# ayushpradhan-dev/robust-speech-analysis-framework

Hardware: AMD Instinct MI355X
Metric: audio-seconds processed/sec (extract+CNN-LSTM fwd) (higher is better)
Workload: dtype f32

## Files before the change

robust_speech_analysis_framework_amd/csrc/gemm_f16x3.h:

```cpp
#pragma once
#if defined(__HIPCC__)
#include "gemm_f32.h"
#define H3_HD __host__ __device__ inline
#else
#include <cstdint>
#define H3_HD inline
#endif

namespace rsaf {

struct H3Div { unsigned mul; int shift; };
inline H3Div h3_div_make(int d) {
    int l = 0;
    while ((1LL << l) < d) ++l;
    const uint64_t two = 1ULL << (31 + l);
    H3Div r;
    r.mul = (unsigned)((two + (uint64_t)d - 1) / (uint64_t)d);
    r.shift = 31 + l;
    return r;
}
H3_HD int h3_div(int n, H3Div r) { return (int)(((uint64_t)(unsigned)n * r.mul) >> r.shift); }
inline bool h3_div_check(H3Div r, int d, int nmax) {
    if (d <= 0 || nmax < 0 || (uint64_t)r.mul * (uint64_t)d < (1ULL << r.shift)) return false;
    const int64_t top = (int64_t)(nmax / d) * d;
// ... 17 lines not shown
    int64_t c_plane, ldcp, sCp;
    const float* c_scale;
    int c_scale_zs, c_scale_ms;
    unsigned* amax_out;
    int amax_zs;
    const int* amax_row_slot;
    int amax_col_min;
    const float* bias;
    const float* R;
    int64_t ldr, sR;
    int M, N, K, nz;
    const int64_t* ztab;
    const int* row_tab;
    int act;
    float alpha;
    int group_m;
    int a_panel, b_panel, cp_panel;
    int nz2;
    int64_t sA2, sB2, sC2, sBias2;
    int b_panel_rows;
    int a_panel_rows, a_tap_panels, a_tap_inv;
    int tiles_m, tiles_n, nwg;
    H3Div inv_nwg, inv_nz2, inv_per_group, inv_gsz, inv_gsz_last;
};

struct H3Tile { int z, z1, z2, tm, tn; };
H3_HD H3Tile h3_tile_at(const GemmH3Params& p, int t) {
    H3Tile T;
    T.z = h3_div(t, p.inv_nwg);
    const int orig = t - T.z * p.nwg;
    T.z1 = h3_div(T.z, p.inv_nz2);
    T.z2 = T.z - T.z1 * (p.nz2 > 1 ? p.nz2 : 1);
    const int xcd = orig & 7, q8 = p.nwg >> 3, r8 = p.nwg & 7;
    const int wg = (xcd < r8 ? xcd * (q8 + 1) : r8 * (q8 + 1) + (xcd - r8) * q8) + (orig >> 3);
    const int per_group = p.group_m * p.tiles_n;
    const int grp = h3_div(wg, p.inv_per_group);
    const int first_m = grp * p.group_m;
    const bool full = p.tiles_m - first_m >= p.group_m;
    const int gsz = full ? p.group_m : p.tiles_m - first_m;
    const int in_grp = wg - grp * per_group;
    T.tn = h3_div(in_grp, full ? p.inv_gsz : p.inv_gsz_last);
    T.tm = first_m + (in_grp - T.tn * gsz);
    return T;
}
inline bool h3_grid_fill(GemmH3Params& p, int bm, int bn) {
    const int64_t tn = (p.N + bn - 1) / bn, tm = (p.M + bm - 1) / bm;
    if (tn <= 0 || tm <= 0 || p.nz <= 0 || p.group_m <= 0 || tn * tm * p.nz > 0x7fffffffLL || p.group_m * tn > 0x7fffffffLL) return false;
    p.tiles_m = (int)tm; p.tiles_n = (int)tn; p.nwg = (int)(tm * tn);
    const int nz2 = p.nz2 > 1 ? p.nz2 : 1, per_group = (int)(p.group_m * tn);
    const int last = p.tiles_m % p.group_m ? p.tiles_m % p.group_m : p.group_m;
    p.inv_nwg = h3_div_make(p.nwg); p.inv_nz2 = h3_div_make(nz2); p.inv_per_group = h3_div_make(per_group);
    p.inv_gsz = h3_div_make(p.group_m); p.inv_gsz_last = h3_div_make(last);
    return h3_div_check(p.inv_nwg, p.nwg, (int)(tm * tn * p.nz - 1)) && h3_div_check(p.inv_nz2, nz2, p.nz - 1) &&
           h3_div_check(p.inv_per_group, per_group, p.nwg - 1) && h3_div_check(p.inv_gsz, p.group_m, per_group - 1) &&
           h3_div_check(p.inv_gsz_last, last, per_group - 1);
}

struct H3KStep { int64_t step, jump; int wrap; };
H3_HD H3KStep h3_kstep(int64_t kstride, int tap_panels, int unit) {
    H3KStep s;
    s.step = kstride * unit;
    s.jump = tap_panels > 0 ? (16 - (int64_t)(tap_panels - 1) * kstride) * unit : s.step;
    s.wrap = tap_panels > 0 ? tap_panels : 0x7fffffff;
    return s;
}
H3_HD int64_t h3_kstep_next(const H3KStep& s, int& pc) {
    const bool w = pc + 1 == s.wrap;
    pc = w ? 0 : pc + 1;
    return w ? s.jump : s.step;
}

#if defined(__HIPCC__)
int launch_gemm_f16x3(const GemmH3Params& p, hipStream_t stream, const char* tag);

int launch_f16x2_row_scales(const float* src, int64_t rows, int K, int64_t ld, float* scale, float* norm2, unsigned* stat_max,
                            hipStream_t stream);
int launch_split_f16x2(const float* src, int64_t rows, int K, int64_t ld, const float* scale, int scale_stride, uint16_t* planes,
                       int64_t plane_stride, int panels, hipStream_t stream);
int launch_scale_from_bound(const unsigned* amax_bits, int64_t n, const float* factor_dev, float factor_host, const float* add_dev,
                            float* scale, hipStream_t stream);

H3_HD float f16x2_scale_for_bound(float bound) {
    union { float f; unsigned u; } v;
    v.f = bound;
    const int e = (int)((v.u >> 23) & 0xff);
    if (e == 0) return 1.0f;
// ... 46 lines not shown
```

robust_speech_analysis_framework_amd/csrc/gemm_f16x3.hip:

```cpp
#include <algorithm>
#include <type_traits>

#include "gemm_f16x3.h"

namespace rsaf {

using f32x16 = __attribute__((ext_vector_type(16))) float;
using f16x8 = __attribute__((ext_vector_type(8))) _Float16;
typedef __attribute__((address_space(3))) void* lds_ptr3;
typedef const __attribute__((address_space(1))) void* glb_ptr3;

__device__ __forceinline__ unsigned short f16_bits(_Float16 h) { return __builtin_bit_cast(unsigned short, h); }

__device__ __forceinline__ void split2(float xs, unsigned short& h, unsigned short& l) {
    const _Float16 hh = (_Float16)xs;
    const _Float16 ll = (_Float16)(xs - (float)hh);
    h = f16_bits(hh);
    l = f16_bits(ll);
}

template <int TM_, int TN_, int WM_, int WN_, int NST_, int WGS_>
struct H3Cfg {
    static constexpr int TM = TM_, TN = TN_, WM = WM_, WN = WN_, NST = NST_, WGS = WGS_;
    static constexpr int BM = 32 * TM * WM, BN = 32 * TN * WN, BK = 16, NPL = 2;
// ... 43 lines not shown
            if (T.m0 < T.Mz) {
                T.coff = p.ztab ? p.ztab[2 * W.z1 + 1] : -1;
                T.aoff = W.z1 * p.sA + W.z2 * p.sA2 + (int64_t)T.m0 * (p.a_panel ? 16 : p.lda);
                T.boff = W.z2 * p.sB2 + (int64_t)T.n0 * (p.b_panel ? 16 : p.ldb);
                T.t = t; T.valid = true;
                break;
            }
        }
        return T;
    };

    constexpr int NI = CFG::A_INSTR + CFG::B_INSTR;
    constexpr int IPW = (NI + NW - 1) / NW;
    constexpr int A_SLOTS = CFG::A_INSTR / NW;
    constexpr int LAST_LIVE = NI - NW * (IPW - 1);
    static_assert(CFG::A_INSTR % NW == 0, "a slot is an A or a B instruction for every wave alike");
    static_assert(LAST_LIVE == NW || LAST_LIVE <= NW / 2, "the waves of group B have the same number of DMA instructions");
    const bool last_live = LAST_LIVE == NW || wave < LAST_LIVE;
#define H3_LIVE(i) ((i) < IPW - 1 || last_live)
    const char* src[IPW][NPL];
    unsigned voff[IPW];
    int ldsoff[IPW];
    int pc = 0;
    const H3KStep a_step = h3_kstep(p.a_panel ? (int64_t)(p.a_panel_rows > 0 ? p.a_panel_rows : p.M) * 16 : 16, p.a_tap_panels, 2);
    const int64_t b_step = 2 * (p.b_panel ? (int64_t)(p.b_panel_rows > 0 ? p.b_panel_rows : p.N) * 16 : 16);
#pragma unroll
    for (int i = 0; i < IPW; ++i) {
        const int jj = i < A_SLOTS ? wave + NW * i : wave + NW * i - CFG::A_INSTR;
        ldsoff[i] = i < A_SLOTS ? jj * 512 : NPL * A_PLANE + jj * 512;
    }
    auto set_tile = [&](const Tile& T) {
        pc = 0;
#pragma unroll
        for (int i = 0; i < IPW; ++i) {
            const bool isA = i < A_SLOTS;
            const int jj = isA ? wave + NW * i : wave + NW * i - CFG::A_INSTR;
            const int row = 32 * jj + (lane >> 1);
            const int dch = (lane & 1) ^ ((row >> 3) & 1);
            const int rr = isA ? ((T.m0 + row < T.Mz) ? row : T.Mz - 1 - T.m0)
                               : ((T.n0 + row < p.N) ? row : p.N - 1 - T.n0);
            const int64_t rs = isA ? (p.a_panel ? 16 : p.lda) : (p.b_panel ? 16 : p.ldb);
            voff[i] = 2u * ((unsigned)rr * (unsigned)rs + 8u * dch);
            const unsigned short* base = isA ? p.A + T.aoff : p.B + T.boff;
#pragma unroll
            for (int pl = 0; pl < NPL; ++pl)
                src[i][pl] = reinterpret_cast<const char*>(base + pl * (isA ? p.a_plane : p.b_plane));
        }
// ... 234 lines not shown
                        const gelu_f32x2 g2 = gelu_pair(gelu_f32x2{v[q][j - 1], v[q][j]});
                        v[q][j - 1] = g2.x; v[q][j] = g2.y;
                    }
                    if (ACT != ACT_NONE && (j & 3) == 3) __builtin_amdgcn_sched_barrier(0);
                }
            }
            if (HAS_R && sub < LAST) load_r((sub + 1) / TN, (sub + 1) % TN);
#pragma unroll
            for (int q = 0; q < NQ; ++q) {
                const int row = drow[q];
                const bool ok = c_ok && tm + RPI * q + lr < Mz && (!ROWTAB || row >= 0);
                if (p.amax_out && ok && gc >= p.amax_col_min) {
#pragma unroll
                    for (int j = 0; j < CW; ++j) row_amax[q] = fmaxf(row_amax[q], fabsf(v[q][j]));
                }
                if (ok) {
                    if (OUT_F32 && p.C) *reinterpret_cast<float4*>(p.C + (done.coff >= 0 ? done.coff : z1 * p.sC) + z2 * p.sC2 + (int64_t)row * p.ldc + gc) =
                        make_float4(v[q][0], v[q][1], v[q][2], v[q][3]);
                    if (OUT_PLANES && p.Cp) {
                        const float cs = csc[q];
                        unsigned short hh[CW], ll[CW];
#pragma unroll
                        for (int j = 0; j < CW; ++j) split2(v[q][j] * cs, hh[j], ll[j]);
                        unsigned short* Pt = p.cp_panel ? p.Cp + (int64_t)(gc >> 4) * ((int64_t)p.M * 16) + (int64_t)row * 16 + (gc & 15)
                                                        : p.Cp + z * p.sCp + (int64_t)row * p.ldcp + gc;
                        if (CW == 8) {
                            *reinterpret_cast<uint4*>(Pt) = make_uint4(hh[0] | ((unsigned)hh[1] << 16), hh[2] | ((unsigned)hh[3] << 16),
                                                                      hh[4 % CW] | ((unsigned)hh[5 % CW] << 16), hh[6 % CW] | ((unsigned)hh[7 % CW] << 16));
                            *reinterpret_cast<uint4*>(Pt + p.c_plane) = make_uint4(ll[0] | ((unsigned)ll[1] << 16), ll[2] | ((unsigned)ll[3] << 16),
                                                                                  ll[4 % CW] | ((unsigned)ll[5 % CW] << 16), ll[6 % CW] | ((unsigned)ll[7 % CW] << 16));
                        } else {
                            *reinterpret_cast<uint2*>(Pt) = make_uint2(hh[0] | ((unsigned)hh[1] << 16), hh[2] | ((unsigned)hh[3] << 16));
                            *reinterpret_cast<uint2*>(Pt + p.c_plane) = make_uint2(ll[0] | ((unsigned)ll[1] << 16), ll[2] | ((unsigned)ll[3] << 16));
                        }
                    }
                }
            }
        }
        if (p.amax_out) {
#pragma unroll
            for (int q = 0; q < NQ; ++q) {
                const int row = tm + RPI * q + lr;
                const bool r_ok = row < Mz && (!ROWTAB || drow[q] >= 0);
                const int slot = !r_ok ? -1 : ROWTAB ? tab_slot[wm0 + mt * 32 + RPI * q + lr]
                                                     : (int)(z1 * p.amax_zs) + (p.amax_row_slot ? p.amax_row_slot[row] : 0);
                unsigned long long todo = __ballot(r_ok);
                while (todo) {
                    const int first = __ffsll((long long)todo) - 1;
// ... 115 lines not shown
    return RSAF_OK;
}

int launch_gemm_f16x3(const GemmH3Params& p, hipStream_t stream, const char* tag) {
    RSAF_CHECK_ARG(p.M >= 0 && p.N >= 0 && p.K >= 0 && p.nz >= 0, "negative dimension");
    if (p.M == 0 || p.N == 0 || p.nz == 0) return RSAF_OK;
    RSAF_CHECK_ARG(p.A && p.B && (p.C || p.Cp), "NULL operand");
    RSAF_CHECK_ARG(p.a_scale && p.b_scale && (!p.Cp || p.c_scale), "every plane operand needs its scales");
    RSAF_CHECK_ARG(p.K % 16 == 0 && p.K >= 16, "K must be a positive multiple of 16");
    RSAF_CHECK_ARG(p.N % 16 == 0, "N must be a multiple of 16 (16-byte epilogue stores)");
    RSAF_CHECK_ARG(p.ldc % 8 == 0 && p.ldcp % 8 == 0 && p.ldr % 4 == 0 && p.c_plane % 8 == 0 && p.sC % 4 == 0 && p.sCp % 8 == 0 &&
                   p.sR % 4 == 0 && p.sC2 % 4 == 0, "ldc / ldr / output strides must keep 16-byte alignment");
    RSAF_CHECK_ARG(p.lda % 8 == 0 && p.ldb % 8 == 0 && p.a_plane % 8 == 0 && p.b_plane % 8 == 0 && p.sA % 8 == 0 && p.sA2 % 8 == 0 &&
                   p.sB2 % 8 == 0, "lda, ldb, the plane strides and the batch strides must be multiples of 8 elements");
    RSAF_CHECK_ARG((reinterpret_cast<uintptr_t>(p.A) & 15) == 0 && (reinterpret_cast<uintptr_t>(p.B) & 15) == 0 &&
                   (reinterpret_cast<uintptr_t>(p.b_scale) & 15) == 0 && p.sBias2 % 4 == 0, "A, B and b_scale must be 16-byte aligned");
    RSAF_CHECK_ARG(!p.R || p.ldr > 0, "residual needs ldr");
    RSAF_CHECK_ARG(p.act >= 0 && p.act <= 2, "act must be 0 (none), 1 (gelu) or 2 (silu)");
    RSAF_CHECK_ARG(p.nz <= 65535, "at most 65535 batches per launch");
    RSAF_CHECK_ARG(!p.cp_panel || p.nz == 1, "the panel layout of the plane output is for unbatched operands");
    RSAF_CHECK_ARG(!p.a_panel || p.nz == 1 || p.a_panel_rows > 0, "a batched A in panels needs a_panel_rows");
    RSAF_CHECK_ARG(p.a_tap_panels == 0 || (p.a_panel && p.a_panel_rows > 0 && p.a_tap_panels > 0 && (p.K / 16) % p.a_tap_panels == 0),
                   "a_tap_panels: A in panels with a_panel_rows, K = taps x a_tap_panels x 16");
    RSAF_CHECK_ARG(p.ldc < (1 << 24) && p.ldcp < (1 << 24) && p.ldr < (1 << 24), "leading dimensions must be below 2^24");
    RSAF_CHECK_ARG(!p.R || p.C, "the residual comes with the fp32 output");
    RSAF_CHECK_ARG(!p.row_tab || (p.nz == 1 && !p.ztab && p.nz2 <= 1 && !p.cp_panel && !p.a_panel && !p.amax_row_slot),
                   "a row table: one batch, row-major A and plane output, no ztab / amax_row_slot");
    RSAF_CHECK_ARG(p.nz2 <= 1 || (p.C && !p.Cp && !p.R && (!p.a_panel || p.a_panel_rows > 0) && p.nz % p.nz2 == 0),
                   "two-level batches: fp32 output only, no residual, A row-major or panels with a_panel_rows, nz a multiple of nz2");
    ProfScope prof(tag ? tag : "gemm_f16x3", stream, 2.0 * p.M * (double)p.N * p.K * p.nz, 0.0);
    using CfgA = H3Cfg<4, 2, 2, 4, 3, 1>;
    using CfgN = H3Cfg<2, 1, 4, 2, 3, 1>;
    using CfgM = H3Cfg<4, 2, 4, 2, 3, 1>;
#define H3_LAUNCH_CFG(CFG, ACT, F32, PL, HR, ...)                                                                       \
    do {                                                                                                                \
        RSAF_CHECK_HIP(hipFuncSetAttribute((const void*)gemm_f16x3_kernel<CFG, ACT, F32, PL, HR, ##__VA_ARGS__>,         \
                                           hipFuncAttributeMaxDynamicSharedMemorySize, CFG::LDS_BYTES));                 \
        RSAF_CHECK_ARG(h3_grid_fill(pp, CFG::BM, CFG::BN), "too many tiles");                                           \
        const int64_t tiles = (int64_t)pp.nwg * pp.nz;                                                                  \
        hipLaunchKernelGGL((gemm_f16x3_kernel<CFG, ACT, F32, PL, HR, ##__VA_ARGS__>),                                    \
                           dim3((unsigned)std::min<int64_t>(tiles, persistent_wgs)), dim3(CFG::THREADS), CFG::LDS_BYTES, stream, pp); \
    } while (0)
#define H3_LAUNCH(ACT, F32, PL, HR, ...)                                                                                \
    do {                                                                                                                \
        if (p.N <= 64) H3_LAUNCH_CFG(CfgN, ACT, F32, PL, HR, ##__VA_ARGS__);                                             \
        else H3_LAUNCH_CFG(CfgA, ACT, F32, PL, HR, ##__VA_ARGS__);                                                       \
    } while (0)
#define H3_LAUNCH3(ACT, F32, PL, HR)                                                                                    \
    do {                                                                                                                \
        if (p.N <= 64) H3_LAUNCH_CFG(CfgN, ACT, F32, PL, HR);                                                            \
// ... 74 lines not shown
```

robust_speech_analysis_framework_amd/csrc/w2v2.hip:

```cpp
#include "w2v2_forward.h"

namespace rsaf {
namespace w2v2 {

int Forward::gemm3(const GemmA& A, const GemmB& B, const Out& o, int M, int N, int K, int nz, const int64_t* zt) {
    GemmH3Params p{};
    p.a_panel = A.panel; p.b_panel = 1; p.cp_panel = o.cp_panel;
    p.A = A.planes; p.a_plane = A.plane; p.lda = A.lda; p.sA = A.sA; p.a_scale = A.scale; p.a_scale_zs = A.scale_zs; p.a_scale_ms = A.scale_ms;
    p.B = B.planes; p.b_plane = (int64_t)N * K; p.ldb = 16; p.b_scale = B.scale;
    p.C = o.Cf; p.ldc = N; p.sC = o.sC;
    p.Cp = o.Cp; p.c_plane = o.c_plane; p.ldcp = N; p.sCp = o.sCp; p.c_scale = o.c_scale; p.c_scale_zs = o.cs_zs; p.c_scale_ms = o.cs_ms;
    p.amax_out = o.amax; p.amax_zs = o.amax_zs; p.amax_row_slot = o.amax_row_slot; p.amax_col_min = o.amax_col_min;
    p.bias = o.bias; p.R = o.R; p.ldr = N; p.sR = o.sC;
    p.M = M; p.N = N; p.K = K; p.nz = nz; p.ztab = zt; p.row_tab = o.row_tab; p.act = o.act; p.alpha = 1.0f; p.group_m = 0;
    return launch_gemm_f16x3(p, s, "w2v2_gemm");
}
GemmA Forward::rows_a(int64_t planes_off, int K, const float* row_scale) const {
    GemmA A;
    A.planes = planes_at(planes_off); A.plane = rows * K; A.lda = K; A.scale = row_scale; A.scale_ms = 1; A.panel = true;
    return A;
}
GemmA Forward::conv_a(const uint16_t* planes, int i) const {
    GemmA A;
    A.planes = planes; A.plane = (int64_t)G * T[i - 1] * C; A.lda = (int64_t)STRD[i] * C; A.sA = (int64_t)T[i - 1] * C;
    A.scale = cscale + (int64_t)(i - 1) * G; A.scale_zs = 1;
    return A;
}
GemmA Forward::conv_a_packed(const uint16_t* planes, int64_t plane, int i) const {
    GemmA A;
    A.planes = planes; A.plane = plane; A.lda = (int64_t)STRD[i] * C;
    A.scale = cscale + (int64_t)(i - 1) * G;
    return A;
}
GemmB Forward::weights_b(int64_t planes_off, int64_t scale_off) const { return GemmB{planes_at(planes_off), ws + scale_off}; }

int Forward::split_wp(int64_t src_off, int64_t nrows, int K, int64_t dst_off, int64_t scale_off, int stat_idx) {
    RSAF_TRY(launch_f16x2_row_scales(Wt + src_off, nrows, K, K, ws + scale_off, nullptr, wstat(stat_idx), s));
    return launch_split_f16x2(Wt + src_off, nrows, K, K, ws + scale_off, 1, planes_at(dst_off), nrows * K, 1, s);
}
int Forward::weight_planes() {
    RSAF_CHECK_HIP(hipMemsetAsync(ws + W.wstat, 0, sizeof(float) * 2 * (WSTAT_LAYER0 + WSTAT_PER_LAYER * c.L), s));
    for (int i = 0; i < 6; ++i)
        RSAF_TRY(split_wp(L.conv[i], C, KERN[i + 1] * C, W.wp_conv[i], W.ws_conv[i], wstat_conv(i)));
    RSAF_TRY(split_wp(L.fpw, Hd, C, W.wp_fp, W.ws_fp, WSTAT_FP));
    if (c.pos_depth() ? posstack_on_mfma(c) : posconv_on_f16x3(c)) {
        RSAF_TRY(split_wp(L.posw, Hd, c.PK * (Hd / c.PG), W.wp_pos, W.ws_pos, WSTAT_POS));
    }
    for (size_t i = 0; i < W.wp_stack.size(); ++i) {
        const int K = c.PK * (Hd / c.PG);
        RSAF_TRY(launch_f16x2_row_scales(Wt + L.stackw[i], Hd, K, K, ws + W.ws_stack[i], nullptr, nullptr, s));
        RSAF_TRY(launch_split_f16x2(Wt + L.stackw[i], Hd, K, K, ws + W.ws_stack[i], 1, planes_at(W.wp_stack[i]), (int64_t)Hd * K, 1, s));
    }
    for (int l = 0; l < c.L; ++l) {
        const LayerOff& lo = L.layers[l];
// ... 195 lines not shown
```

robust_speech_analysis_framework_amd/csrc/w2v2_feat.hip:

```cpp
#include "w2v2_forward.h"
#include "gn_stats.h"

namespace rsaf {
namespace w2v2 {

__global__ __launch_bounds__(256) void w2v2_tables_kernel(const int* __restrict__ len, int n, int C, int Hd, int* __restrict__ Tw,
                                                          int64_t* __restrict__ row0, int64_t* __restrict__ ztab) {
    for (int w = threadIdx.x; w < n; w += 256) {
        int m = len[w];
        for (int i = 0; i < 7; ++i) { m = m >= KERN[i] ? (m - KERN[i]) / STRD[i] + 1 : 0; Tw[(int64_t)i * n + w] = m; }
    }
    __syncthreads();
    if (threadIdx.x == 0) {
        int64_t r = 0;
        for (int w = 0; w < n; ++w) { row0[w] = r; r += Tw[(int64_t)6 * n + w]; }
        row0[n] = r;
    }
    __syncthreads();
    for (int w = threadIdx.x; w < n; w += 256) {
        for (int j = 0; j < 5; ++j) { ztab[((int64_t)j * n + w) * 2] = Tw[(int64_t)(j + 1) * n + w]; ztab[((int64_t)j * n + w) * 2 + 1] = -1; }
        ztab[((int64_t)5 * n + w) * 2] = Tw[(int64_t)6 * n + w]; ztab[((int64_t)5 * n + w) * 2 + 1] = row0[w] * C;
        ztab[((int64_t)6 * n + w) * 2] = Tw[(int64_t)6 * n + w]; ztab[((int64_t)6 * n + w) * 2 + 1] = row0[w] * Hd;
    }
}
// ... 114 lines not shown
            const int64_t o = (2 * (int64_t)out_off[chunk] + t) * C + ch[0];
            if (CPT % 2 == 0) {
#pragma unroll
                for (int k = 0; k < CPT; k += 2) {
                    *reinterpret_cast<unsigned*>(outp + o + k) = hh[k] | ((unsigned)hh[k + 1] << 16);
                    *reinterpret_cast<unsigned*>(outp + plane + o + k) = ll[k] | ((unsigned)ll[k + 1] << 16);
                }
            } else {
#pragma unroll
                for (int k = 0; k < CPT; ++k) { outp[o + k] = hh[k]; outp[plane + o + k] = ll[k]; }
            }
        }
    }
    if (!APPLY) {
#pragma unroll
        for (int k = 0; k < CPT; ++k) {
            part[(((int64_t)chunk * slabs + sl) * 3 + 0) * C + ch[k]] = s[k];
            part[(((int64_t)chunk * slabs + sl) * 3 + 1) * C + ch[k]] = q[k];
            part[(((int64_t)chunk * slabs + sl) * 3 + 2) * C + ch[k]] = mx[k];
        }
    }
}

__global__ __launch_bounds__(384) void lnconv_scale_kernel(const float* __restrict__ cln, int C, int G, float* __restrict__ scale) {
    const int i = threadIdx.x >> 6, lane = threadIdx.x & 63;
    const float* g = cln + (int64_t)2 * i * C;
    const float* b = g + C;
    float mg = 0.f, mb = 0.f;
    for (int c = lane; c < C; c += 64) { mg = fmaxf(mg, fabsf(g[c])); mb = fmaxf(mb, fabsf(b[c])); }
#pragma unroll
    for (int o = 32; o >= 1; o >>= 1) { mg = fmaxf(mg, __shfl_xor(mg, o, 64)); mb = fmaxf(mb, __shfl_xor(mb, o, 64)); }
    const float bound = fmaxf(mg * sqrtf((float)C) * 1.0001f + mb, 0.17f) * 1.0001f;
    const float sc = f16x2_scale_for_bound(bound);
    for (int w = lane; w < G; w += 64) scale[(int64_t)i * G + w] = sc;
}

__global__ __launch_bounds__(64) void conv_bias_max_kernel(const float* __restrict__ cb, int C, float* __restrict__ out) {
    for (int i = 1; i < 6; ++i) {
        float m = 0.f;
        for (int c = threadIdx.x; c < C; c += 64) m = fmaxf(m, fabsf(cb[(int64_t)i * C + c]));
#pragma unroll
        for (int o = 32; o >= 1; o >>= 1) m = fmaxf(m, __shfl_xor(m, o, 64));
        if (threadIdx.x == 0) out[i] = m * 1.000001f;
    }
}

// ... 139 lines not shown
#pragma unroll
        for (int j = 0; j < 10; ++j) wr[j] = w0[c * 10 + j];
        const float bi = cb ? cb[c] : 0.f;
        gn::Sums64 acc;
        for (int t = 0; t < T0; ++t) {
            float y = 0.f;
#pragma unroll
            for (int j = 0; j < 10; ++j) y = fmaf(wr[j], x[5 * t + j], y);
            if (cb) y += bi;
            acc.add(y);
        }
        m = gn::moments_of_sums(acc.s, acc.q, T0);
    }
    float af, bf;
    gn::coefficients(m, g[c], be[c], af, bf);
    ab[((int64_t)chunk * 2 + 0) * C + c] = af;
    ab[((int64_t)chunk * 2 + 1) * C + c] = bf;
    atomicMax(amax + chunk, __float_as_uint((fabsf(af) * mx + fabsf(bf)) * 1.000001f));
}

template <bool APPLY>
static int conv0_launch(const Cfg& c, const float* xn, const float* w0, const float* cb, float* part, const float* ab, const float* scale,
                        unsigned short* outp, int64_t plane, int n, int len, const int* T0w, const int* out_off, int T0, int slab, int slabs,
                        hipStream_t s) {
    const int threads = c.C <= 256 ? c.C : 256;
    const int cpt = c.C / threads;
    dim3 grid((unsigned)slabs, (unsigned)n);
    ProfScope prof(APPLY ? "w2v2_conv0_apply" : "w2v2_conv0_stats", s, 0.0,
                   APPLY ? (double)n * ((double)c.C * T0 * 4.0 + 4.0 * (5.0 * T0 + 5.0)) : (double)n * 4.0 * (5.0 * T0 + 5.0));
#define RSAF_C0K(CPT, BIAS)                                                                                \
    hipLaunchKernelGGL((conv0_kernel<CPT, APPLY, BIAS>), grid, dim3(threads), 0, s, xn, w0, cb, part, ab, scale, outp, plane, len, T0w, \
                       out_off, c.C, slab, slabs)
#define RSAF_C0(BIAS)                                                                                      \
    switch (cpt) {                                                                                         \
        case 1: RSAF_C0K(1, BIAS); break;                                                                  \
        case 2: RSAF_C0K(2, BIAS); break;                                                                  \
        case 3: RSAF_C0K(3, BIAS); break;                                                                  \
        case 4: RSAF_C0K(4, BIAS); break;                                                                  \
        default: set_error("conv0: unsupported conv_dim"); return RSAF_ERR_ARG;                            \
    }
    if (cb) { RSAF_C0(true) } else { RSAF_C0(false) }
#undef RSAF_C0
#undef RSAF_C0K
    RSAF_CHECK_HIP(hipGetLastError());
    return RSAF_OK;
}

static int conv0_ln_launch(const Cfg& c, const float* xn, const float* w0, const float* cb, const float* lg, const float* lb,
                           const float* scale, unsigned short* outp, int64_t plane, int n, int len, const int* T0w, int T0,
                           int T0g, hipStream_t s) {
    constexpr int FR = 64;
    dim3 grid((unsigned)((T0g + FR - 1) / FR), (unsigned)n);
    ProfScope prof("w2v2_conv0_ln", s, 0.0, (double)n * ((double)c.C * T0g * 4.0 + 4.0 * (5.0 * T0g + 5.0)));
    const int cpt = (c.C + 63) / 64;
#define RSAF_C0L(CPT)                                                                                                      \
    hipLaunchKernelGGL((conv0_ln_kernel<CPT>), grid, dim3(256), 0, s, xn, w0, cb, lg, lb, scale, outp, plane, len, T0w, T0, \
                       c.C, FR)
    switch (cpt) {
        case 1: RSAF_C0L(1); break;
        case 2: RSAF_C0L(2); break;
        case 3: RSAF_C0L(3); break;
        case 4: RSAF_C0L(4); break;
        case 8: RSAF_C0L(8); break;
        case 12: RSAF_C0L(12); break;
// ... 63 lines not shown
            hipLaunchKernelGGL(conv_ln_gelu_kernel, dim3((unsigned)((lrows + 3) / 4)), dim3(256), 0, s, ws + W.Q,
                               cln + (int64_t)2 * i * C, cln + (int64_t)(2 * i + 1) * C, cscale + (int64_t)i * G,
                               planes_at(W.P), (int64_t)G * T[i] * C, lrows, T[i], Tw + (int64_t)i * n + g0, C);
            RSAF_CHECK_HIP(hipGetLastError());
        }
    }
    return RSAF_OK;
}
int Forward::convs_group_norm(int g0, int g, const int* Tg) {
    int64_t M[7] = {};
    for (int w = g0; w < g0 + g; ++w) {
        int Tw_[7];
        chunk_lengths(R.len[w], Tw_);
        for (int i = 1; i < 7; ++i) M[i] += Tw_[i] + 1;
    }
    RSAF_CHECK_ARG(2 * M[1] + 1 < 0x7fffffffLL && rows < 0x7fffffffLL, "too many conv rows in one group");
    PackBases bases{};
    for (int i = 1; i < 7; ++i) bases.b[i] = packed_tab_base(G, T, i);
    hipLaunchKernelGGL(w2v2_pack_offsets_kernel, dim3(1), dim3(64), 0, s, Tw + g0, n, g, G, coff);
    hipLaunchKernelGGL(w2v2_pack_rows_kernel, dim3(g, 6), dim3(256), 0, s, Tw + g0, n, G, coff, row0 + g0, crow, bases);
    RSAF_CHECK_HIP(hipGetLastError());
    const int slabs_g = (Tg[0] + STAT_SLAB - 1) / STAT_SLAB;
    RSAF_TRY(conv0_launch<false>(c, ws + W.xn, Wt + L.conv0, cbias, ws + W.part, nullptr, nullptr, nullptr, 0, g, R.maxlen, Tw + g0,
                                  nullptr, T[0], STAT_SLAB, slabs_g, s));
    const int64_t tot = (int64_t)g * C;
    hipLaunchKernelGGL(gn_finalize_kernel, dim3((unsigned)((tot + 255) / 256)), dim3(256), 0, s, ws + W.part,
                       Wt + L.gng, Wt + L.gnb, ws + W.ab, camax, g, C, slabs_g, Tw + g0, ws + W.xn, R.maxlen, Wt + L.conv0, cbias);
    RSAF_CHECK_HIP(hipGetLastError());
    RSAF_TRY(launch_scale_from_bound(camax, g, nullptr, 1.0f, nullptr, cscale, s));
    const int slab = 128;
    const int64_t plane_p = p_rows(G, T) * C, plane_q = q_rows(G, T) * C;
    RSAF_TRY(conv0_launch<true>(c, ws + W.xn, Wt + L.conv0, cbias, nullptr, ws + W.ab, cscale, planes_at(W.P), plane_p, g,
                                 R.maxlen, Tw + g0, coff + (G + 1), T[0], slab, (Tg[0] + slab - 1) / slab, s));
    uint16_t* cur = planes_at(W.P);
    uint16_t* nxt = planes_at(W.Q);
    int64_t plane_cur = plane_p, plane_nxt = plane_q;
    for (int i = 1; i < 7; ++i) {
        Out o;
        o.act = ACT_GELU;
        o.row_tab = crow + 2 * bases.b[i];
        if (i < 6) {
            RSAF_TRY(launch_scale_from_bound(camax + (int64_t)(i - 1) * G, g, reinterpret_cast<const float*>(wstat(wstat_conv(i - 1))),
                                              sqrtf((float)(KERN[i] * C)) * 1.00001f, conv_bias ? cb_max + i : nullptr,
                                              cscale + (int64_t)i * G, s));
            o.Cp = nxt; o.c_plane = plane_nxt;
            o.c_scale = cscale + (int64_t)i * G;
            o.amax = camax + (int64_t)i * G;
        } else {
            o.Cf = ws + W.c6;
        }
        o.bias = conv_bias ? cbias + (int64_t)i * C : nullptr;
        RSAF_TRY(gemm3(conv_a_packed(cur, plane_cur, i), weights_b(W.wp_conv[i - 1], W.ws_conv[i - 1]), o, (int)M[i], C, KERN[i] * C));
        std::swap(cur, nxt);
        std::swap(plane_cur, plane_nxt);
    }
    return RSAF_OK;
}

int Forward::feature_projection() {
    RSAF_CHECK_HIP(hipMemsetAsync(ws + W.fp_amax, 0, sizeof(unsigned) * n, s));
    LnArgs a;
    a.x = ws + W.c6; a.g = Wt + L.fplg; a.b = Wt + L.fplb;
    a.planes = planes_at(W.lnfp); a.panel = true; a.scale_out = ws + W.s_lnfp;
    if (layer_norm) {
        a.var = 2; a.pg = cln + (int64_t)12 * C; a.pb = cln + (int64_t)13 * C;
    } else if (c.flags & F_NO_FEAT_PROJ_LN) {
        a.var = 3;
    }
    RSAF_TRY(ln(a, rows, C, c.eps, s));
    Out o;
    o.Cf = x; o.bias = Wt + L.fpb;
    o.amax = bits_at(W.fp_amax); o.amax_row_slot = rowwin;
    return gemm3(rows_a(W.lnfp, C, ws + W.s_lnfp), weights_b(W.wp_fp, W.ws_fp), o, (int)rows, Hd, C);
}

// ... 3 lines not shown
```

robust_speech_analysis_framework_amd/csrc/w2v2_forward.h:

```cpp
#pragma once
#include <algorithm>
#include <cstdlib>
#include <vector>

#include "gemm_f32.h"
#include "gemm_f16x3.h"
#include "w2v2_layout.h"

namespace rsaf {
namespace w2v2 {

__device__ __forceinline__ unsigned short f16_bits_w(_Float16 h) { return __builtin_bit_cast(unsigned short, h); }
__device__ __forceinline__ void split2_w(float xs, unsigned short& h, unsigned short& l) {
    const _Float16 hh = (_Float16)xs;
    h = f16_bits_w(hh);
    l = f16_bits_w((_Float16)(xs - (float)hh));
}

#define RSAF_TRY(expr) do { const int rc_ = (expr); if (rc_) return rc_; } while (0)

struct LnArgs {
    const float *x = nullptr, *r = nullptr;
    const float *g = nullptr, *b = nullptr;
    float* out = nullptr;
// ... 2 lines not shown
    const int64_t* row0 = nullptr;
    unsigned short* planes = nullptr;
    bool panel = false;
    float* scale_out = nullptr;
    const unsigned *bound_w = nullptr, *bound_b = nullptr;
    float* bound_scale_out = nullptr;
    unsigned* win_norm = nullptr;
    int var = 0;
    const float *pg = nullptr, *pb = nullptr;
    float* aux = nullptr;
    float* tap = nullptr;
    int tap_mode = 0;
    const int64_t* tap_row_start = nullptr;
};

int ln(const LnArgs& a, int64_t rows, int D, float eps, hipStream_t s);

struct GemmA {
    const uint16_t* planes = nullptr;
    int64_t plane = 0, lda = 0, sA = 0;
    const float* scale = nullptr;
    int scale_zs = 0, scale_ms = 0;
    bool panel = false;
};
struct GemmB {
    const uint16_t* planes = nullptr;
    const float* scale = nullptr;
};
struct Out {
    const float* bias = nullptr;
    const float* R = nullptr;
    int act = ACT_NONE;
    float* Cf = nullptr;
    int64_t sC = 0;
    uint16_t* Cp = nullptr;
    int64_t c_plane = 0, sCp = 0;
    const float* c_scale = nullptr;
    int cs_zs = 0, cs_ms = 0;
    bool cp_panel = false;
    unsigned* amax = nullptr;
    int amax_zs = 0;
    const int* amax_row_slot = nullptr;
    int amax_col_min = 0;
    const int* row_tab = nullptr;
};

struct Forward {
    const Cfg& c;
    const Rag& R;
    const Layout L;
    const Workspace& W;
    const float* Wt;
    float* ws;
    hipStream_t s;
    const float* wav = nullptr;
    const int64_t* chunk_start = nullptr;
    float* out = nullptr;
    const int64_t* out_row_start = nullptr;
    float* const* taps = nullptr;
    const int n, C, Hd, Tt, G, hd;
    const int* T;
    const int64_t rows;
// ... 14 lines not shown
    float* x;

    Forward(const Cfg& c_, const Rag& R_, const Workspace& W_, const float* weights, void* workspace, hipStream_t s_)
        : c(c_), R(R_), L(make_layout(c_)), W(W_), Wt(weights), ws(static_cast<float*>(workspace)), s(s_), n(R_.n), C(c_.C), Hd(c_.Hd),
          Tt(R_.Tmax[6]), G(conv_group(R_.n)), hd(c_.Hd / c_.NH), T(R_.Tmax), rows(R_.rows), scale(1.0f / sqrtf((float)hd)),
          fused(fused_attention(c_, Tt)), relpos(c_.flags & F_REL_POS_BIAS), pre_ln(c_.flags & F_PRE_LN),
          layer_norm(c_.flags & F_LAYER_FEAT_NORM), conv_bias(c_.flags & F_CONV_BIAS),
          Tw(reinterpret_cast<int*>(ws + W.t_Tw)), row0(reinterpret_cast<int64_t*>(ws + W.t_row0)),
          ztab(reinterpret_cast<int64_t*>(ws + W.t_ztab)), rowwin(reinterpret_cast<int*>(ws + W.t_rowwin)),
          coff(reinterpret_cast<int*>(ws + W.t_coff)), crow(reinterpret_cast<int*>(ws + W.t_crow)),
          cscale(ws + W.conv_scale), camax(bits_at(W.conv_amax)), cbias(conv_bias ? Wt + L.cb : nullptr), cln(Wt + L.cln),
          cb_max(conv_bias ? ws + W.cb_max : nullptr), x(ws + W.x) {}

    uint16_t* planes_at(int64_t off) const { return reinterpret_cast<uint16_t*>(ws + off); }
    unsigned* bits_at(int64_t off) const { return reinterpret_cast<unsigned*>(ws + off); }
    unsigned* wstat(int idx) const { return bits_at(W.wstat) + 2 * idx; }
    float* tap(int k) const { return taps ? taps[k] : nullptr; }
    float* gate_rows() const { return relpos ? ws + W.att : nullptr; }
    float* gate() const { return relpos ? ws + W.gate : nullptr; }
    const float* reltab() const { return relpos ? Wt + L.reltab : nullptr; }

    int gemm3(const GemmA& A, const GemmB& B, const Out& o, int M, int N, int K, int nz = 1, const int64_t* zt = nullptr);
    GemmA rows_a(int64_t planes_off, int K, const float* row_scale) const, conv_a(const uint16_t* planes, int i) const,
        conv_a_packed(const uint16_t* planes, int64_t plane, int i) const;
    GemmB weights_b(int64_t planes_off, int64_t scale_off) const;
    int split_wp(int64_t src_off, int64_t nrows, int K, int64_t dst_off, int64_t scale_off, int stat_idx), weight_planes();
    int window_tables(const int* len_dev), feature_encoder(), conv_gemm(int i, const uint16_t* a_planes, Out& o, int g0, int g, const int* Tg),
        convs_layer_norm(int g0, int g, const int* Tg), convs_group_norm(int g0, int g, const int* Tg), feature_projection();
    int positional_conv(), positional_conv_stack(), posstack_mfma(int D), posstack_fp32(int D), posconv_regroup_planes(), posconv_lds(),
        posconv_batched_gemm(),
        conv_runs_fp32(const float* src, const float* w, const float* bias, int act, const char* gemm_family, const char* regroup_family);
    template <int MODE> int posstack_rows(const float* src, float* dst);
    template <int NT> int posstack_conv_launch(int i);
    template <int NT, int SP> int posconv_lds_launch();
    int ln_to_qkv(const float* src, const float* res, const float* g, const float* b, float* dst, int k, bool next, float* sum = nullptr);
    int qkv_projection(int l), attention(), attention_three_launch(), out_projection(int l),
        ln_to_ffn(int l, const float* g, const float* b, float* dst), feed_forward(int l, float* dst, const float* res), layer_post_ln(int l),
        layer_pre_ln(int l), encoder_layer(int l);
    template <bool RP> int attention_fused();
};

}
}
```

robust_speech_analysis_framework_amd/csrc/w2v2_layout.h:

```cpp
#pragma once
#include <cstddef>
#include <cstdint>
#include <utility>
#include <vector>

#include "rsaf.h"

#if defined(__HIPCC__)
#define WL_HD __host__ __device__ __forceinline__
#else
#define WL_HD inline
#endif

namespace rsaf {
namespace w2v2 {

constexpr int F_LAYER_FEAT_NORM = RSAF_W2V2_LAYER_FEAT_NORM, F_CONV_BIAS = RSAF_W2V2_CONV_BIAS, F_PRE_LN = RSAF_W2V2_PRE_LN,
              F_NO_INPUT_NORM = RSAF_W2V2_NO_INPUT_NORM, F_NO_FEAT_PROJ_LN = RSAF_W2V2_NO_FEAT_PROJ_LN,
              F_REL_POS_BIAS = RSAF_W2V2_REL_POS_BIAS, F_POS_CONV_STACK = RSAF_W2V2_POS_CONV_STACK,
              F_POS_DEPTH_MASK = RSAF_W2V2_POS_DEPTH_MASK,
              F_ALL = 15 | F_NO_FEAT_PROJ_LN | F_REL_POS_BIAS | F_POS_CONV_STACK | F_POS_DEPTH_MASK;
constexpr int REL_SPAN = RSAF_W2V2_REL_SPAN, REL_TAB = 2 * REL_SPAN - 1;

struct Cfg {
// ... 97 lines not shown
    std::vector<int64_t> wp_qkv, wp_o, wp_1, wp_2;
    int64_t ws_conv[6], ws_fp, ws_pos, wstat;
    std::vector<int64_t> ws_qkv, ws_o, ws_1, ws_2;
    int64_t conv_scale, conv_amax, pos_scale, fp_amax, wlen, win_norm, s_lnfp, s_x, s_ffn, s_att, s_qkv;
    int64_t cb_max;
    int64_t gate;
    std::vector<int64_t> wp_stack, ws_stack;
    int64_t t_Tw, t_row0, t_ztab, t_rowwin;
    int64_t t_coff, t_crow;
};
constexpr int STAT_SLAB = 512;
constexpr int CONV_GROUP = 512;

inline int conv_group(int n) { return n < CONV_GROUP ? n : CONV_GROUP; }
inline bool fused_attention(const Cfg& c, int Tt) { return c.Hd / c.NH == 64 && Tt <= 256; }
inline bool posconv_on_f16x3(const Cfg& c) { return (c.Hd / c.PG) % 16 == 0; }
inline bool posstack_on_mfma(const Cfg& c) { return c.pos_depth() > 0 && (c.Hd / c.PG) % 16 == 0 && c.Hd / c.PG <= 64; }

inline int64_t planes_floats(int64_t n) { return pad4(n); }

inline int64_t packed_in_rows(int G, int Ti) { return 2 * (int64_t)G * (Ti + 1) + 1; }
inline int64_t p_rows(int G, const int* T) { return packed_in_rows(G, T[1]); }
inline int64_t q_rows(int G, const int* T) { return packed_in_rows(G, T[2]); }
inline int64_t packed_tab_base(int G, const int* T, int i) {
    int64_t b = 0;
    for (int j = 1; j < i; ++j) b += (int64_t)G * (T[j] + 1);
    return b;
}

inline int wstat_conv(int i) { return i; }
constexpr int WSTAT_FP = 6, WSTAT_POS = 7, WSTAT_LAYER0 = 8, WSTAT_PER_LAYER = 6;

struct Rag {
    int n = 0, maxlen = 0, Tmax[7] = {};
    int64_t rows = 0;
    std::vector<int> len;
    std::vector<int64_t> row0;
    std::vector<std::pair<int, int>> tgroups;
    std::vector<int> T6;
};

inline const char* make_rag(const int* len_host, int n, int len, Rag& R) {
    R.n = n;
    if (len_host) R.len.assign(len_host, len_host + n);
    else R.len.assign((size_t)n, len);
    R.row0.assign(n + 1, 0);
// ... 113 lines not shown
```

Baseline: 12550.

## Store feature-encoder conv activations as even/odd panel images for strided conv GEMMs

Switches the f16x3 plane layout of the strided feature-encoder convolutions from row-major packed rows to a 16-wide panel layout split into even-row and odd-row images. The GEMM epilogue writes the next layer's A operand directly in this layout, and the A loader's k-step walks across two (or three) taps over the image pair, so the stride-2 conv A tiles become contiguous panel loads. Conv layers after the first use the new layout by default. An opt-in conv0 kernel, enabled by an environment variable, stages outputs in LDS and writes the panels itself. This adds layout complexity and argument checks, and carries a risk of indexing mistakes with odd T lengths.

```diff
diff --git a/robust_speech_analysis_framework_amd/csrc/gemm_f16x3.h b/robust_speech_analysis_framework_amd/csrc/gemm_f16x3.h
--- a/robust_speech_analysis_framework_amd/csrc/gemm_f16x3.h
+++ b/robust_speech_analysis_framework_amd/csrc/gemm_f16x3.h
@@ -63,7 +63,12 @@
     int a_panel_rows, a_tap_panels, a_tap_inv;
     int tiles_m, tiles_n, nwg;
     H3Div inv_nwg, inv_nz2, inv_per_group, inv_gsz, inv_gsz_last;
+    int a_evenodd, cp_evenodd_rows;
 };
+
+H3_HD int64_t h3_evenodd_at(int64_t R, int P, int r, int k) {
+    return (((int64_t)(r & 1) * P + (k >> 4)) * R + (r >> 1)) * 16 + (k & 15);
+}
 
 struct H3Tile { int z, z1, z2, tm, tn; };
 H3_HD H3Tile h3_tile_at(const GemmH3Params& p, int t) {
@@ -98,11 +103,12 @@
 }
 
 struct H3KStep { int64_t step, jump; int wrap; };
-H3_HD H3KStep h3_kstep(int64_t kstride, int tap_panels, int unit) {
+H3_HD H3KStep h3_kstep(int64_t kstride, int tap_panels, int unit, int images = 1) {
     H3KStep s;
+    const int per_wrap = tap_panels * images;
     s.step = kstride * unit;
-    s.jump = tap_panels > 0 ? (16 - (int64_t)(tap_panels - 1) * kstride) * unit : s.step;
-    s.wrap = tap_panels > 0 ? tap_panels : 0x7fffffff;
+    s.jump = tap_panels > 0 ? (16 - (int64_t)(per_wrap - 1) * kstride) * unit : s.step;
+    s.wrap = tap_panels > 0 ? per_wrap : 0x7fffffff;
     return s;
 }
 H3_HD int64_t h3_kstep_next(const H3KStep& s, int& pc) {
diff --git a/robust_speech_analysis_framework_amd/csrc/gemm_f16x3.hip b/robust_speech_analysis_framework_amd/csrc/gemm_f16x3.hip
--- a/robust_speech_analysis_framework_amd/csrc/gemm_f16x3.hip
+++ b/robust_speech_analysis_framework_amd/csrc/gemm_f16x3.hip
@@ -89,7 +89,8 @@
     unsigned voff[IPW];
     int ldsoff[IPW];
     int pc = 0;
-    const H3KStep a_step = h3_kstep(p.a_panel ? (int64_t)(p.a_panel_rows > 0 ? p.a_panel_rows : p.M) * 16 : 16, p.a_tap_panels, 2);
+    const H3KStep a_step = h3_kstep(p.a_panel ? (int64_t)(p.a_panel_rows > 0 ? p.a_panel_rows : p.M) * 16 : 16, p.a_tap_panels, 2,
+                                    (ROWTAB && p.a_evenodd) ? 2 : 1);
     const int64_t b_step = 2 * (p.b_panel ? (int64_t)(p.b_panel_rows > 0 ? p.b_panel_rows : p.N) * 16 : 16);
 #pragma unroll
     for (int i = 0; i < IPW; ++i) {
@@ -370,8 +371,9 @@
                         unsigned short hh[CW], ll[CW];
 #pragma unroll
                         for (int j = 0; j < CW; ++j) split2(v[q][j] * cs, hh[j], ll[j]);
-                        unsigned short* Pt = p.cp_panel ? p.Cp + (int64_t)(gc >> 4) * ((int64_t)p.M * 16) + (int64_t)row * 16 + (gc & 15)
-                                                        : p.Cp + z * p.sCp + (int64_t)row * p.ldcp + gc;
+                        unsigned short* Pt = (ROWTAB && p.cp_panel) ? p.Cp + h3_evenodd_at(p.cp_evenodd_rows, p.N >> 4, row, gc)
+                                             : p.cp_panel ? p.Cp + (int64_t)(gc >> 4) * ((int64_t)p.M * 16) + (int64_t)row * 16 + (gc & 15)
+                                                          : p.Cp + z * p.sCp + (int64_t)row * p.ldcp + gc;
                         if (CW == 8) {
                             *reinterpret_cast<uint4*>(Pt) = make_uint4(hh[0] | ((unsigned)hh[1] << 16), hh[2] | ((unsigned)hh[3] << 16),
                                                                       hh[4 % CW] | ((unsigned)hh[5 % CW] << 16), hh[6 % CW] | ((unsigned)hh[7 % CW] << 16));
@@ -533,10 +535,15 @@
     RSAF_CHECK_ARG(!p.a_panel || p.nz == 1 || p.a_panel_rows > 0, "a batched A in panels needs a_panel_rows");
     RSAF_CHECK_ARG(p.a_tap_panels == 0 || (p.a_panel && p.a_panel_rows > 0 && p.a_tap_panels > 0 && (p.K / 16) % p.a_tap_panels == 0),
                    "a_tap_panels: A in panels with a_panel_rows, K = taps x a_tap_panels x 16");
+    RSAF_CHECK_ARG(!p.a_evenodd || (p.row_tab && p.a_tap_panels > 0 && (p.K / 16 == 2 * p.a_tap_panels || p.K / 16 == 3 * p.a_tap_panels) &&
+                                    p.M <= p.a_panel_rows),
+                   "a_evenodd: a row table, A as two images of a_tap_panels panels x a_panel_rows >= M rows, 2 or 3 taps");
+    RSAF_CHECK_ARG(p.cp_evenodd_rows >= 0 && (p.cp_evenodd_rows > 0) == (p.row_tab && p.cp_panel && p.Cp),
+                   "cp_evenodd_rows comes with a row table and the panel layout of the plane output, and they with it");
     RSAF_CHECK_ARG(p.ldc < (1 << 24) && p.ldcp < (1 << 24) && p.ldr < (1 << 24), "leading dimensions must be below 2^24");
     RSAF_CHECK_ARG(!p.R || p.C, "the residual comes with the fp32 output");
-    RSAF_CHECK_ARG(!p.row_tab || (p.nz == 1 && !p.ztab && p.nz2 <= 1 && !p.cp_panel && !p.a_panel && !p.amax_row_slot),
-                   "a row table: one batch, row-major A and plane output, no ztab / amax_row_slot");
+    RSAF_CHECK_ARG(!p.row_tab || (p.nz == 1 && !p.ztab && p.nz2 <= 1 && (!p.a_panel || p.a_evenodd) && !p.amax_row_slot),
+                   "a row table: one batch, A row-major or an even / odd image pair, no ztab / amax_row_slot");
     RSAF_CHECK_ARG(p.nz2 <= 1 || (p.C && !p.Cp && !p.R && (!p.a_panel || p.a_panel_rows > 0) && p.nz % p.nz2 == 0),
                    "two-level batches: fp32 output only, no residual, A row-major or panels with a_panel_rows, nz a multiple of nz2");
     ProfScope prof(tag ? tag : "gemm_f16x3", stream, 2.0 * p.M * (double)p.N * p.K * p.nz, 0.0);
diff --git a/robust_speech_analysis_framework_amd/csrc/w2v2.hip b/robust_speech_analysis_framework_amd/csrc/w2v2.hip
--- a/robust_speech_analysis_framework_amd/csrc/w2v2.hip
+++ b/robust_speech_analysis_framework_amd/csrc/w2v2.hip
@@ -13,6 +13,8 @@
     p.amax_out = o.amax; p.amax_zs = o.amax_zs; p.amax_row_slot = o.amax_row_slot; p.amax_col_min = o.amax_col_min;
     p.bias = o.bias; p.R = o.R; p.ldr = N; p.sR = o.sC;
     p.M = M; p.N = N; p.K = K; p.nz = nz; p.ztab = zt; p.row_tab = o.row_tab; p.act = o.act; p.alpha = 1.0f; p.group_m = 0;
+    if (A.evenodd_rows > 0) { p.a_evenodd = 1; p.a_panel_rows = A.evenodd_rows; p.a_tap_panels = A.evenodd_panels; }
+    p.cp_evenodd_rows = o.cp_evenodd_rows;
     return launch_gemm_f16x3(p, s, "w2v2_gemm");
 }
 GemmA Forward::rows_a(int64_t planes_off, int K, const float* row_scale) const {
@@ -26,10 +28,11 @@
     A.scale = cscale + (int64_t)(i - 1) * G; A.scale_zs = 1;
     return A;
 }
-GemmA Forward::conv_a_packed(const uint16_t* planes, int64_t plane, int i) const {
+GemmA Forward::conv_a_packed(const uint16_t* planes, int64_t plane, int i, bool evenodd) const {
     GemmA A;
     A.planes = planes; A.plane = plane; A.lda = (int64_t)STRD[i] * C;
     A.scale = cscale + (int64_t)(i - 1) * G;
+    if (evenodd) { A.panel = true; A.lda = 16; A.evenodd_rows = (int)evenodd_img_rows(G, T[i]); A.evenodd_panels = C / 16; }
     return A;
 }
 GemmB Forward::weights_b(int64_t planes_off, int64_t scale_off) const { return GemmB{planes_at(planes_off), ws + scale_off}; }
diff --git a/robust_speech_analysis_framework_amd/csrc/w2v2_feat.hip b/robust_speech_analysis_framework_amd/csrc/w2v2_feat.hip
--- a/robust_speech_analysis_framework_amd/csrc/w2v2_feat.hip
+++ b/robust_speech_analysis_framework_amd/csrc/w2v2_feat.hip
@@ -160,6 +160,69 @@
     }
 }
 
+constexpr int C0P_CH = 128, C0P_FR = 64, C0P_ROWB = C0P_CH * 2 + 16;
+template <bool BIAS>
+__global__ __launch_bounds__(256) void conv0_panels_kernel(const float* __restrict__ xn, const float* __restrict__ w0,
+                                                           const float* __restrict__ cb, const float* __restrict__ ab,
+                                                           const float* __restrict__ scale, unsigned short* __restrict__ outp,
+                                                           int64_t plane, int len, const int* __restrict__ T0w,
+                                                           const int* __restrict__ out_off, int C, int slab, int rimg) {
+    __shared__ __attribute__((aligned(16))) unsigned char stage[2 * C0P_FR * C0P_ROWB];
+    const int chunk = blockIdx.y, lane = threadIdx.x & 63, wave = __builtin_amdgcn_readfirstlane(threadIdx.x >> 6);
+    const int t0 = blockIdx.x * slab, t1 = min(T0w[chunk], t0 + slab);
+    const int c0 = blockIdx.z * C0P_CH, nch = min(C - c0, C0P_CH);
+    const bool live = 2 * lane < nch;
+    const int ch = c0 + (live ? 2 * lane : 0);
+    const float* __restrict__ x = xn + (int64_t)chunk * len;
+    float wr[2][10], a[2], b[2], bi[2];
+    const float sc = scale[chunk];
+#pragma unroll
+    for (int k = 0; k < 2; ++k) {
+#pragma unroll
+        for (int j = 0; j < 10; ++j) wr[k][j] = w0[(ch + k) * 10 + j];
+        bi[k] = BIAS ? cb[ch + k] : 0.f;
+        a[k] = ab[((int64_t)chunk * 2 + 0) * C + ch + k]; b[k] = ab[((int64_t)chunk * 2 + 1) * C + ch + k];
+    }
+    const int np = nch >> 4;
+    const int64_t r0 = 2 * (int64_t)out_off[chunk];
+    const int rr = lane >> 1, half = lane & 1;
+    const int lane_src = 2 * rr * C0P_ROWB + 16 * half, lane_dst = 16 * rr + 8 * half;
+    for (int tb = t0; tb < t1; tb += C0P_FR) {
+        for (int tt = 16 * wave; tt < 16 * wave + 16 && tb + tt < t1; ++tt) {
+            const int t = tb + tt;
+            float xv[10], gv[2];
+#pragma unroll
+            for (int j = 0; j < 10; ++j) xv[j] = x[5 * t + j];
+#pragma unroll
+            for (int k = 0; k < 2; ++k) {
+                float y = 0.f;
+#pragma unroll
+                for (int j = 0; j < 10; ++j) y = fmaf(wr[k][j], xv[j], y);
+                if (BIAS) y += bi[k];
+                gv[k] = fmaf(y, a[k], b[k]);
+            }
+            const gelu_f32x2 g2 = gelu_pair(gelu_f32x2{gv[0], gv[1]});
+            unsigned short hh[2], ll[2];
+            split2_w(g2.x * sc, hh[0], ll[0]);
+            split2_w(g2.y * sc, hh[1], ll[1]);
+            if (live) {
+                *reinterpret_cast<unsigned*>(stage + tt * C0P_ROWB + 4 * lane) = hh[0] | ((unsigned)hh[1] << 16);
+                *reinterpret_cast<unsigned*>(stage + (C0P_FR + tt) * C0P_ROWB + 4 * lane) = ll[0] | ((unsigned)ll[1] << 16);
+            }
+        }
+        __syncthreads();
+#pragma unroll
+        for (int w = 0; w < 4; ++w) {
+            const int img = w & 1, pl = w >> 1;
+            if (tb + 2 * rr + img < t1)
+                for (int panel = wave; panel < np; panel += 4)
+                    *reinterpret_cast<uint4*>(outp + pl * plane + evenodd_at(rimg, C, r0 + tb + img, c0 + 16 * panel) + lane_dst) =
+                        *reinterpret_cast<const uint4*>(stage + (pl * C0P_FR + img) * C0P_ROWB + 32 * panel + lane_src);
+        }
+        __syncthreads();
+    }
+}
+
 __global__ __launch_bounds__(384) void lnconv_scale_kernel(const float* __restrict__ cln, int C, int G, float* __restrict__ scale) {
     const int i = threadIdx.x >> 6, lane = threadIdx.x & 63;
     const float* g = cln + (int64_t)2 * i * C;
@@ -345,7 +408,7 @@
 template <bool APPLY>
 static int conv0_launch(const Cfg& c, const float* xn, const float* w0, const float* cb, float* part, const float* ab, const float* scale,
                         unsigned short* outp, int64_t plane, int n, int len, const int* T0w, const int* out_off, int T0, int slab, int slabs,
-                        hipStream_t s) {
+                        int rimg, hipStream_t s) {
     const int threads = c.C <= 256 ? c.C : 256;
     const int cpt = c.C / threads;
     dim3 grid((unsigned)slabs, (unsigned)n);
@@ -362,7 +425,11 @@
         case 4: RSAF_C0K(4, BIAS); break;                                                                  \
         default: set_error("conv0: unsupported conv_dim"); return RSAF_ERR_ARG;                            \
     }
-    if (cb) { RSAF_C0(true) } else { RSAF_C0(false) }
+    if (APPLY && rimg > 0) {
+        dim3 pgrid((unsigned)slabs, (unsigned)n, (unsigned)((c.C + C0P_CH - 1) / C0P_CH));
+        if (cb) hipLaunchKernelGGL(conv0_panels_kernel<true>, pgrid, dim3(256), 0, s, xn, w0, cb, ab, scale, outp, plane, len, T0w, out_off, c.C, slab, rimg);
+        else hipLaunchKernelGGL(conv0_panels_kernel<false>, pgrid, dim3(256), 0, s, xn, w0, cb, ab, scale, outp, plane, len, T0w, out_off, c.C, slab, rimg);
+    } else if (cb) { RSAF_C0(true) } else { RSAF_C0(false) }
 #undef RSAF_C0
 #undef RSAF_C0K
     RSAF_CHECK_HIP(hipGetLastError());
@@ -472,16 +539,19 @@
     RSAF_CHECK_HIP(hipGetLastError());
     const int slabs_g = (Tg[0] + STAT_SLAB - 1) / STAT_SLAB;
     RSAF_TRY(conv0_launch<false>(c, ws + W.xn, Wt + L.conv0, cbias, ws + W.part, nullptr, nullptr, nullptr, 0, g, R.maxlen, Tw + g0,
-                                  nullptr, T[0], STAT_SLAB, slabs_g, s));
+                                  nullptr, T[0], STAT_SLAB, slabs_g, 0, s));
     const int64_t tot = (int64_t)g * C;
     hipLaunchKernelGGL(gn_finalize_kernel, dim3((unsigned)((tot + 255) / 256)), dim3(256), 0, s, ws + W.part,
                        Wt + L.gng, Wt + L.gnb, ws + W.ab, camax, g, C, slabs_g, Tw + g0, ws + W.xn, R.maxlen, Wt + L.conv0, cbias);
     RSAF_CHECK_HIP(hipGetLastError());
     RSAF_TRY(launch_scale_from_bound(camax, g, nullptr, 1.0f, nullptr, cscale, s));
-    const int slab = 128;
     const int64_t plane_p = p_rows(G, T) * C, plane_q = q_rows(G, T) * C;
+    const auto env1 = [](const char* name) { const char* e = getenv(name); return e && e[0] == '1'; };
+    const bool evenodd = !env1("RSAF_W2V2_CONV_ROWMAJOR"), evenodd0 = evenodd && env1("RSAF_W2V2_CONV0_PANELS");
+    const int slab = evenodd0 ? 512 : 128;
     RSAF_TRY(conv0_launch<true>(c, ws + W.xn, Wt + L.conv0, cbias, nullptr, ws + W.ab, cscale, planes_at(W.P), plane_p, g,
-                                 R.maxlen, Tw + g0, coff + (G + 1), T[0], slab, (Tg[0] + slab - 1) / slab, s));
+                                 R.maxlen, Tw + g0, coff + (G + 1), T[0], slab, (Tg[0] + slab - 1) / slab,
+                                 evenodd0 ? (int)evenodd_img_rows(G, T[1]) : 0, s));
     uint16_t* cur = planes_at(W.P);
     uint16_t* nxt = planes_at(W.Q);
     int64_t plane_cur = plane_p, plane_nxt = plane_q;
@@ -494,13 +564,14 @@
                                               sqrtf((float)(KERN[i] * C)) * 1.00001f, conv_bias ? cb_max + i : nullptr,
                                               cscale + (int64_t)i * G, s));
             o.Cp = nxt; o.c_plane = plane_nxt;
+            if (evenodd) { o.cp_panel = true; o.cp_evenodd_rows = (int)evenodd_img_rows(G, T[i + 1]); }
             o.c_scale = cscale + (int64_t)i * G;
             o.amax = camax + (int64_t)i * G;
         } else {
             o.Cf = ws + W.c6;
         }
         o.bias = conv_bias ? cbias + (int64_t)i * C : nullptr;
-        RSAF_TRY(gemm3(conv_a_packed(cur, plane_cur, i), weights_b(W.wp_conv[i - 1], W.ws_conv[i - 1]), o, (int)M[i], C, KERN[i] * C));
+        RSAF_TRY(gemm3(conv_a_packed(cur, plane_cur, i, i > 1 ? evenodd : evenodd0), weights_b(W.wp_conv[i - 1], W.ws_conv[i - 1]), o, (int)M[i], C, KERN[i] * C));
         std::swap(cur, nxt);
         std::swap(plane_cur, plane_nxt);
     }
diff --git a/robust_speech_analysis_framework_amd/csrc/w2v2_forward.h b/robust_speech_analysis_framework_amd/csrc/w2v2_forward.h
--- a/robust_speech_analysis_framework_amd/csrc/w2v2_forward.h
+++ b/robust_speech_analysis_framework_amd/csrc/w2v2_forward.h
@@ -48,6 +48,7 @@
     const float* scale = nullptr;
     int scale_zs = 0, scale_ms = 0;
     bool panel = false;
+    int evenodd_rows = 0, evenodd_panels = 0;
 };
 struct GemmB {
     const uint16_t* planes = nullptr;
@@ -64,6 +65,7 @@
     const float* c_scale = nullptr;
     int cs_zs = 0, cs_ms = 0;
     bool cp_panel = false;
+    int cp_evenodd_rows = 0;
     unsigned* amax = nullptr;
     int amax_zs = 0;
     const int* amax_row_slot = nullptr;
@@ -124,7 +126,7 @@
 
     int gemm3(const GemmA& A, const GemmB& B, const Out& o, int M, int N, int K, int nz = 1, const int64_t* zt = nullptr);
     GemmA rows_a(int64_t planes_off, int K, const float* row_scale) const, conv_a(const uint16_t* planes, int i) const,
-        conv_a_packed(const uint16_t* planes, int64_t plane, int i) const;
+        conv_a_packed(const uint16_t* planes, int64_t plane, int i, bool evenodd) const;
     GemmB weights_b(int64_t planes_off, int64_t scale_off) const;
     int split_wp(int64_t src_off, int64_t nrows, int K, int64_t dst_off, int64_t scale_off, int stat_idx), weight_planes();
     int window_tables(const int* len_dev), feature_encoder(), conv_gemm(int i, const uint16_t* a_planes, Out& o, int g0, int g, const int* Tg),
diff --git a/robust_speech_analysis_framework_amd/csrc/w2v2_layout.h b/robust_speech_analysis_framework_amd/csrc/w2v2_layout.h
--- a/robust_speech_analysis_framework_amd/csrc/w2v2_layout.h
+++ b/robust_speech_analysis_framework_amd/csrc/w2v2_layout.h
@@ -143,6 +143,11 @@
 inline int64_t packed_in_rows(int G, int Ti) { return 2 * (int64_t)G * (Ti + 1) + 1; }
 inline int64_t p_rows(int G, const int* T) { return packed_in_rows(G, T[1]); }
 inline int64_t q_rows(int G, const int* T) { return packed_in_rows(G, T[2]); }
+WL_HD int64_t evenodd_img_rows(int G, int Ti) { return (int64_t)G * (Ti + 1); }
+WL_HD int64_t evenodd_plane_elems(int G, int Ti, int C) { return 2 * evenodd_img_rows(G, Ti) * C; }
+WL_HD int64_t evenodd_at(int64_t Rimg, int C, int64_t r, int ch) {
+    return ((((r & 1) * (C >> 4)) + (ch >> 4)) * Rimg + (r >> 1)) * 16 + (ch & 15);
+}
 inline int64_t packed_tab_base(int G, const int* T, int i) {
     int64_t b = 0;
     for (int j = 1; j < i; ++j) b += (int64_t)G * (T[j] + 1);
```

After: 12630, median of 6. No clear change (+0.6%).
